# verdurin/pbdagcon

Hardware: AMD Instinct MI355X
Metric: consensus bases/sec (whole node) (higher is better)
Workload: dtype u8

## Files before the change

### include/dagcon.h

```cpp
#ifndef DAGCON_H
#define DAGCON_H

#include <stddef.h>
#include <stdint.h>

#ifdef __cplusplus
extern "C" {
#endif

#define DAGCON_ABI_VERSION 2

typedef enum dagcon_status {
    DAGCON_OK = 0,
    DAGCON_ERR_INVALID_ARG = -1,
    DAGCON_ERR_NO_DEVICE = -2,
    DAGCON_ERR_HIP = -3,
    DAGCON_ERR_NONCONFORMING = -4,
    DAGCON_ERR_UNSUPPORTED = -5,
    DAGCON_ERR_WORKSPACE = -6,
    DAGCON_ERR_INTERNAL = -7,
    DAGCON_ERR_STATE = -8
} dagcon_status;

#define DAGCON_MAX_COVERAGE 4094u
// ... 305 lines not shown
int dagcon_debug_counters(dagcon_ctx *ctx, unsigned long long *out8);

uint32_t dagcon_align_dropped(dagcon_ctx *ctx);

int dagcon_align_ends(dagcon_ctx *ctx, uint32_t n, uint32_t *q_begin, uint32_t *q_end, uint32_t *t_begin,
                      uint32_t *t_end);

#define DAGCON_PLACE_MAX_LEN 65536u
int dagcon_place(dagcon_ctx *ctx, const uint64_t *seq_off, const uint32_t *seq_len, const char *blob, uint64_t bytes,
                 uint32_t n_pairs, const uint32_t *pair_q, const uint32_t *pair_t, uint32_t k, uint32_t max_occ,
                 uint32_t *votes_fwd, uint32_t *votes_rev, char *strand, uint32_t *t0, uint32_t *t1);

int dagcon_debug_plan(uint32_t n_targets, uint64_t n_alignments, uint64_t sum_positions, uint32_t partial_span,
                      uint32_t max_segments, uint32_t min_segment_len, uint32_t out4[4]);

#ifdef __cplusplus
}
#endif
#endif
```

### pbdagcon_amd/capi.py

```python
from __future__ import annotations

import ctypes as C
import os

import numpy as np

_HERE = os.path.dirname(os.path.abspath(__file__))
LIB_PATH = os.path.join(_HERE, "libdagcon_hip.so")

DAGCON_OK = 0
ERR_NAMES = {
    -1: "DAGCON_ERR_INVALID_ARG", -2: "DAGCON_ERR_NO_DEVICE", -3: "DAGCON_ERR_HIP",
    -4: "DAGCON_ERR_NONCONFORMING", -5: "DAGCON_ERR_UNSUPPORTED", -6: "DAGCON_ERR_WORKSPACE",
    -7: "DAGCON_ERR_INTERNAL", -8: "DAGCON_ERR_STATE",
}
FLAG_RAW_ALIGNMENTS = 1
FLAG_STOP_AFTER_BUILD = 2
FLAG_STOP_AFTER_MERGE = 4
FLAG_DEBUG_RESWEEP = 16
FLAG_LOCAL_ALIGN = 32
FLAG_BASE_SUPPORT = 64
FLAG_BASE_POS = 256
MAX_COVERAGE = 4094
PLACE_MAX_LEN = 65536
# ... 5 lines not shown
    "dagcon_debug_counters", "dagcon_host_alloc", "dagcon_host_free", "dagcon_align",
    "dagcon_consensus_pre", "dagcon_debug_plan", "dagcon_align_dropped", "dagcon_align_panels",
    "dagcon_align_ends", "dagcon_place", "dagcon_fetch_support", "dagcon_upload_cigar", "dagcon_consensus_cigar",
    "dagcon_fetch_positions", "dagcon_upload_cigar_windows", "dagcon_consensus_cigar_windows",
    "dagcon_upload_cigar_packed", "dagcon_consensus_cigar_packed",
    "dagcon_upload_cigar_strand", "dagcon_consensus_cigar_strand",
    "dagcon_upload_cs", "dagcon_consensus_cs",
    "dagcon_set_record_filter", "dagcon_fetch_record_stats",
    "dagcon_set_edits", "dagcon_fetch_edits",
    "dagcon_set_edit_support", "dagcon_fetch_edit_support",
    "dagcon_set_pileup", "dagcon_fetch_pileup", "dagcon_fetch_pileup_sites",
    "dagcon_set_site_reads", "dagcon_fetch_site_reads",
    "dagcon_set_site_alleles", "dagcon_fetch_site_alleles", "dagcon_allele_text",
    "dagcon_set_hap_consensus", "dagcon_fetch_hap_tally", "dagcon_upload_haps", "dagcon_fetch_hap_map",
    "dagcon_upload_cigar_md", "dagcon_consensus_cigar_md", "dagcon_fetch_md_targets",
]
ABI_VERSION = 2


class DagconError(RuntimeError):
    def __init__(self, code, msg):
        super().__init__(f"{ERR_NAMES.get(code, code)}: {msg}")
        self.code = code


class Opts(C.Structure):
    _fields_ = [("min_cov", C.c_uint32), ("min_len", C.c_uint32), ("trim", C.c_uint32),
                ("min_weight", C.c_int32), ("device", C.c_int32), ("flags", C.c_uint32),
                ("max_segments", C.c_uint32), ("min_segment_len", C.c_uint32)]

# ... 191 lines not shown
    L.dagcon_fetch_pileup.argtypes = [vp, C.POINTER(Pileup)]
    L.dagcon_fetch_pileup_sites.argtypes = [vp, C.POINTER(PileupSites)]
    L.dagcon_set_site_reads.argtypes = [vp, C.POINTER(SiteReadsOpts)]
    L.dagcon_fetch_site_reads.argtypes = [vp, C.POINTER(SiteReads)]
    L.dagcon_set_site_alleles.argtypes = [vp, C.c_int]
    L.dagcon_fetch_site_alleles.argtypes = [vp, C.POINTER(SiteAlleles)]
    L.dagcon_allele_text.argtypes = [C.c_uint64, C.c_char_p, C.c_size_t]
    L.dagcon_set_hap_consensus.argtypes = [vp, C.POINTER(HapOpts)]
    L.dagcon_fetch_hap_tally.argtypes = [vp, C.POINTER(HapTally)]
    L.dagcon_upload_haps.argtypes = [vp]
    L.dagcon_fetch_hap_map.argtypes = [vp, C.POINTER(HapMap)]
    L.dagcon_upload_cigar_md.argtypes = [vp, C.POINTER(CigarBatch), C.POINTER(Windows), C.POINTER(MdTags), C.c_int]
    L.dagcon_consensus_cigar_md.argtypes = [vp, C.POINTER(CigarBatch), C.POINTER(Windows), C.POINTER(MdTags), C.c_int,
                                            C.POINTER(Results)]
    L.dagcon_fetch_md_targets.argtypes = [vp, C.POINTER(vp), C.POINTER(C.c_uint64)]
    L.dagcon_host_alloc.argtypes = [vp, C.c_size_t, C.POINTER(vp)]
    L.dagcon_host_free.argtypes = [vp, vp]
    L.dagcon_host_free.restype = None
    _LIB = L
    return L


def allele_text(key) -> str:
    buf = C.create_string_buffer(24)
    r = load().dagcon_allele_text(int(key), buf, 24)
    if r != 0:
        raise DagconError(r, "dagcon_allele_text: %#x is no key" % int(key))
    return buf.value.decode()


def default_opts() -> Opts:
    o = Opts()
    load().dagcon_default_opts(C.byref(o))
    return o


class HostBatch:

    def __init__(self, tlen, aln_begin, aln_start, aln_off, aln_len, qstr, tstr,
                 backbone=None, backbone_off=None, ids=None):
        self.tlen = np.ascontiguousarray(tlen, dtype=np.uint32)
        self.aln_begin = np.ascontiguousarray(aln_begin, dtype=np.uint64)
        self.aln_start = np.ascontiguousarray(aln_start, dtype=np.uint32)
# ... 623 lines not shown
        return {"src_target": np.ctypeslib.as_array(hm.src_target, shape=(T,)).copy() if T else np.zeros(0, np.uint32),
                "label": np.ctypeslib.as_array(hm.label, shape=(T,)).copy() if T else np.zeros(0, np.uint8),
                "aln_begin": begin,
                "aln_src": np.ctypeslib.as_array(hm.aln_src, shape=(n,)).copy() if n else np.zeros(0, np.uint64)}

    def edits(self) -> dict:
        e = Edits()
        self._chk(self.L.dagcon_fetch_edits(self.h, C.byref(e)))
        S, n = int(e.n_segments), int(e.n)

        def arr(ptr, k, dt):
            return np.ctypeslib.as_array(ptr, shape=(k,)).copy() if k else np.zeros(0, dt)
        return {"seg_t0": arr(e.seg_t0, S, np.uint32), "seg_t1": arr(e.seg_t1, S, np.uint32),
                "edit_begin": arr(e.edit_begin, S + 1, np.uint64), "t_pos": arr(e.t_pos, n, np.uint32),
                "t_len": arr(e.t_len, n, np.uint32), "c_off": arr(e.c_off, n, np.uint64), "c_len": arr(e.c_len, n, np.uint32)}

    def timings(self) -> dict:
        t = Timings()
        self._chk(self.L.dagcon_get_timings(self.h, C.byref(t)))
        return {k: getattr(t, k) for k, _ in Timings._fields_ if k != "reserved"}

    def normalize(self, alns, trim=0, raw=False):
        n = len(alns)
        starts = np.array([a[0] for a in alns], dtype=np.uint32)
        lens = np.array([len(a[1]) for a in alns], dtype=np.uint32)
        offs = np.zeros(n, dtype=np.uint64)
        if n:
            offs[1:] = np.cumsum(lens[:-1], dtype=np.uint64)
        q = np.frombuffer(b"".join(a[1] for a in alns) or b"\0", dtype=np.uint8)
        t = np.frombuffer(b"".join(a[2] for a in alns) or b"\0", dtype=np.uint8)
# ... 151 lines not shown
```

### pbdagcon_amd/csrc/api_ctx.h

```cpp
namespace {

struct Ctx;

struct DevBuf {
    void *p = nullptr;
    size_t cap = 0;
    DevBuf() = default;
    DevBuf(const DevBuf &) = delete;
    DevBuf &operator=(const DevBuf &) = delete;
    ~DevBuf() { release(); }
    void release() {
        if (p) (void)hipFree(p);
        p = nullptr; cap = 0;
    }
    template <class X> X *as() const { return static_cast<X *>(p); }
};

struct PinBuf {
    void *p = nullptr;
    size_t cap = 0;
    PinBuf() = default;
    PinBuf(const PinBuf &) = delete;
    PinBuf &operator=(const PinBuf &) = delete;
    ~PinBuf() { if (p) (void)hipHostFree(p); }
// ... 106 lines not shown
    uint32_t max_k = 0, max_tlen = 0;
    uint64_t sum_len = 0, sum_bb = 0, mat_cells = 0, blob_bytes = 0;
    bool have_bb = false;
    std::vector<uint32_t> h_tlen, h_aln_len, h_aln_start, h_aln_tgt;
    std::vector<uint64_t> h_aln_begin, h_aln_off, h_mat_base, h_bbv_base, h_bb_off, h_matc_base;
    std::vector<uint32_t> h_matc_stride;
    uint64_t matc_cells = 0;
    bool wide_cells = false;
    std::vector<uint8_t> h_tactive;
    std::vector<uint32_t> h_ch_base, h_ch_aln;
    std::vector<uint64_t> h_norm_off;
    std::vector<uint32_t> h_ck_base;
    uint64_t n_ckpt = 0;
    uint32_t emit_shift = 9;
    uint32_t n_chunks = 0;
    uint64_t tmp_main = 0, tmp_cap = 0;
    bool tmp_shared = false;

    InBufs in;
    RunBufs run;
    ArenaBufs arena;
    AlignBufs al;
    PanelBufs pn;
    PlaceBufs pl;
    CsBufs cs;
    CigarBufs cg;
    MdBufs md;
    bool md_valid = false, md_fetched = false;
    uint64_t md_bytes = 0;
    std::vector<char> h_md_t;
// ... 175 lines not shown
```

### pbdagcon_amd/csrc/api_run.hip.h

```cpp
namespace {

#define DQ_KMAX 52u
struct DgPlanIn { uint32_t T; uint64_t n_alns, sum_bb; uint32_t gcuts, max_segments, min_segment_len, seg_env, merge_q; };
struct DgPlan { uint32_t seg_max, seg_min, use_q, bp_max; };
static DgPlan dg_plan_pieces(const DgPlanIn &in) {
    DgPlan pl;
    const uint32_t T = in.T;
    pl.seg_min = in.min_segment_len;
    if (!pl.seg_min) pl.seg_min = (uint32_t)std::min<uint64_t>(768, std::max<uint64_t>(192, in.sum_bb / 8192));
    if (in.max_segments) pl.seg_max = in.max_segments > 64u ? 64u : in.max_segments;
    else if (in.seg_env) pl.seg_max = in.seg_env;
    else if (in.gcuts) pl.seg_max = 64;
    else { uint32_t sm = T ? 8192u / T : 8u; pl.seg_max = sm < 8u ? 8u : sm > 256u ? 256u : sm; }
    if (in.gcuts && !in.min_segment_len) pl.seg_min = 256;
    pl.use_q = 0;
    if (in.merge_q && !in.gcuts && pl.seg_max != 1) {
        const uint32_t slots = 1024u * DQ_WAVES;
        if (in.max_segments || in.seg_env) pl.use_q = 1;
        else if (T && in.n_alns <= (uint64_t)DQ_KMAX * T) {
            const uint64_t avail = std::min<uint64_t>(256, std::max<uint64_t>(1, in.sum_bb / T / 128));
            const uint64_t k = (uint64_t)T * avail / DQ_ROWS / slots;
            if (k >= 1 || (uint64_t)T * avail / DQ_ROWS * 10u >= 6u * slots) {
                const uint64_t sm = std::min<uint64_t>(avail, std::max<uint64_t>(k, 1) * slots * DQ_ROWS / T);
                if (sm >= 2) { pl.seg_max = (uint32_t)sm; pl.use_q = 1; }
            }
        }
    }
    if (pl.seg_max < 1) pl.seg_max = 1;
    if (pl.use_q && !in.min_segment_len) pl.seg_min = 128;
    pl.bp_max = pl.seg_max == 1 ? 1u : std::min(in.gcuts || T >= 256u ? 64u : (uint32_t)DG_BP_PIECES, 3u * pl.seg_max);
    if (pl.bp_max < 1) pl.bp_max = 1;
    return pl;
}

size_t seg_stride(const Ctx *c) { return ((size_t)c->seg_cap + 3) & ~(size_t)3; }

bool matc_wide(const Ctx *c) { return c->max_k > 64u || c->wide_cells; }
size_t matc_bytes(const Ctx *c) { return (size_t)c->matc_cells * (matc_wide(c) ? 4u : 1u); }

int ensure_stat(Ctx *c, uint32_t T) {
    StatBlock &b = c->sb;
    auto up16 = [](size_t x) { return (x + 15) & ~(size_t)15; };
    b.o_tfail = up16(sizeof(DgStatus));
    b.o_cns_len = b.o_tfail + up16(((size_t)T + 1) * 4);
    b.o_n_seg = b.o_cns_len + up16((size_t)T * 4);
    b.zero_bytes = b.o_n_seg + up16((size_t)T * 4);
    b.o_cns_off = b.zero_bytes;
// ... 99 lines not shown
    p.bb_off = c->in.bb_off.as<const uint64_t>();
    p.mat_base = c->in.mat_base.as<const uint64_t>();
    p.matc_base = c->in.matc_base.as<const uint64_t>(); p.matc_stride = c->in.matc_stride.as<const uint32_t>();
    p.bbv_base = c->in.bbv_base.as<const uint64_t>();
    p.T = c->T; p.A = c->A;
    p.trim = c->opts.trim; p.min_len = c->opts.min_len;
    p.min_weight = c->opts.min_weight < 0 ? (int32_t)c->opts.min_cov : c->opts.min_weight;
    p.flags = c->opts.flags;
    p.max_k = c->max_k; p.max_tlen = c->max_tlen;
    p.nmis = c->run.nmis.as<uint32_t>(); p.norm_off = c->in.norm_off.as<uint64_t>();
    p.n_lo = c->run.n_lo.as<uint32_t>(); p.n_hi = c->run.n_hi.as<uint32_t>();
    p.n_start = c->run.n_start.as<uint32_t>(); p.n_ins = c->run.n_ins.as<uint32_t>();
    p.n_del = c->run.n_del.as<uint32_t>();
    p.norm = c->arena.norm.as<uint16_t>(); p.norm_cap = c->norm_cap;
    p.ch_aln = c->in.ch_aln.as<const uint32_t>(); p.ch_base = c->in.ch_base.as<const uint32_t>();
    p.n_chunks = c->n_chunks;
    p.ch_k0 = c->run.ch_k0.as<uint32_t>(); p.ch_next = c->run.ch_next.as<uint32_t>();
    p.ch_w = c->run.ch_w.as<uint32_t>(); p.ch_tb = c->run.ch_tb.as<uint32_t>();
    p.ch_flag = c->run.ch_flag.as<uint32_t>(); p.ch_src = c->run.ch_src.as<uint64_t>();
    p.ch_out = c->run.ch_out.as<uint32_t>(); p.ch_adv = c->run.ch_adv.as<uint32_t>();
    p.n_lb = c->run.n_lb.as<uint32_t>(); p.norm_tmp = c->run.norm_tmp.as<uint16_t>();
    p.tmp_main = c->tmp_main; p.tmp_cap = c->tmp_cap; p.tmp_off = c->tmp_shared ? c->in.tmp_off.as<const uint64_t>() : nullptr;
    p.ckpt = c->run.ckpt.as<uint32_t>(); p.ck_base = c->in.ck_base.as<const uint32_t>(); p.emit_shift = c->emit_shift;
    p.node_base = c->run.node_base.as<uint64_t>(); p.n_nodes = c->run.n_nodes.as<uint32_t>();
    p.pool_base = c->run.pool_base.as<uint64_t>(); p.pool_size = c->run.pool_size.as<uint32_t>();
    p.pool_top = c->run.pool_top.as<uint32_t>(); p.t_nins = c->run.t_nins.as<uint32_t>();
    p.matA = c->arena.matA.as<uint32_t>(); p.matD = c->arena.matD.as<uint32_t>(); p.matC = c->arena.matC.p;
    p.cov = c->run.cov.as<int32_t>(); p.gcount = c->run.gcount.as<uint32_t>();
    p.gbase = c->run.gbase.as<uint32_t>(); p.bid = c->run.bid.as<uint32_t>();
    p.nodes = c->arena.nodes.as<DgNode>(); p.best = c->run.best.as<int32_t>();
    p.queue = c->run.queue.as<int32_t>(); p.score = c->run.score.as<float2>(); p.bp_tt = c->run.bp_tt.as<float>();
// ... 256 lines not shown
    c->device = opts->device;
    if (const char *e = getenv("DAGCON_EMIT_SHIFT")) {
        const int v = atoi(e);
        if (v >= 4 && v <= 20) c->emit_shift = (uint32_t)v;
    }
    if (const char *e = getenv("DAGCON_MERGE_SEGS")) {
        const int v = atoi(e);
        if (v >= 1 && v <= 64) c->seg_env = (uint32_t)v;
    }
    if (const char *e = getenv("DAGCON_FOLD")) c->fold = atoi(e) != 0;
    if (const char *e = getenv("DAGCON_POISON")) c->poison = atoi(e);
    if (const char *e = getenv("DAGCON_BP_LANE")) c->bp_lane = atoi(e);
    if (const char *e = getenv("DAGCON_BP_LANE_STACK")) c->bl_stk = atoi(e);
    if (const char *e = getenv("DAGCON_MERGE_Q")) c->merge_q = atoi(e) != 0;
    if (const char *e = getenv("DAGCON_EDITS_CAP")) c->ed_cap_env = atol(e);
    memset(&c->tm, 0, sizeof c->tm);
    memset(&c->h_st, 0, sizeof c->h_st);
    if (hipSetDevice(c->device) != hipSuccess || hipStreamCreateWithFlags(&c->stream, hipStreamNonBlocking) != hipSuccess) {
        delete c;
        return DAGCON_ERR_NO_DEVICE;
    }
    for (auto &e : c->ev)
        if (hipEventCreate(&e) != hipSuccess) { delete c; return DAGCON_ERR_HIP; }
    if (ensure_stat(c, 0) != DAGCON_OK) { delete c; return DAGCON_ERR_WORKSPACE; }
    *out = reinterpret_cast<dagcon_ctx *>(c);
    return DAGCON_OK;
}

void dagcon_destroy(dagcon_ctx *ctx) { delete reinterpret_cast<Ctx *>(ctx); }

static bool has_long_gap_run(const char *tstr, const std::vector<uint64_t> &off, const std::vector<uint32_t> &len) {
    for (size_t a = 0; a < len.size(); a++) {
        const char *s = tstr + off[a];
        uint32_t run = 0;
        for (uint32_t i = 0; i < len[a]; i++) {
            run = s[i] == '-' || s[i] == '.' ? run + 1 : 0;
            if (run > 255u) return true;
        }
    }
// ... 75 lines not shown
        c->sum_bb += ((uint64_t)b->tlen[t] + 2 + 3) & ~3ull;
        if (c->have_bb) {
            c->h_bb_off[t] = b->backbone_off[t];
            bb_bytes = std::max<uint64_t>(bb_bytes, b->backbone_off[t] + b->tlen[t]);
        }
    }
    if (was_wide && !dev_t && b->tstr) c->wide_cells = has_long_gap_run(b->tstr, c->h_aln_off, c->h_aln_len);
    c->full_span = n_whole == (uint64_t)c->h_aln_len.size();
    c->gcuts = c->full_span ? 0u : 1u;
    if (const char *e = getenv("DAGCON_GCUTS")) c->gcuts = atoi(e) ? 1u : 0u;
    {
        DgPlanIn pi;
        pi.T = T; pi.n_alns = c->h_aln_len.size(); pi.sum_bb = c->sum_bb; pi.gcuts = c->gcuts;
        pi.max_segments = c->opts.max_segments; pi.min_segment_len = c->opts.min_segment_len;
        pi.seg_env = c->seg_env; pi.merge_q = c->merge_q ? 1u : 0u;
        const DgPlan pl = dg_plan_pieces(pi);
        c->seg_max = pl.seg_max; c->seg_min = pl.seg_min; c->use_q = (int)pl.use_q; c->bp_max = pl.bp_max;
    }
    if (const char *e = getenv("DAGCON_BP_SEGS")) { const int v = atoi(e); if (v >= 1 && v <= 64) c->bp_max = (uint32_t)v; }
    {
        const uint64_t pieces = std::max<uint64_t>(1, (uint64_t)T * std::max(c->bp_max, c->seg_max));
        const uint32_t fit = (uint32_t)std::min<uint64_t>(4096, (512ull << 20) / pieces);
        const uint32_t base = std::max(256u, fit);
        if (c->stk_words < base || (uint64_t)c->stk_words * pieces > (1024ull << 20)) c->stk_words = base;
    }
    if (c->gcuts) c->worklist_cap = std::max<uint32_t>(c->worklist_cap, (uint32_t)std::min<uint64_t>((uint64_t)T * c->seg_max + 64, 0x0FFFFFFFull));
    c->h_aln_begin[T] = c->h_aln_len.size();
    if (c->h_aln_len.size() > 0xFFFFFFF0ull) return fail(c, DAGCON_ERR_UNSUPPORTED, "too many alignments");
    c->A = (uint32_t)c->h_aln_len.size();
    c->blob_bytes = b->blob_bytes;
    c->h_ch_base.assign((size_t)c->A + 1, 0);
    c->h_ch_aln.clear();
    for (uint32_t a = 0; a < c->A; a++) {
        const uint32_t nw = std::max<uint32_t>(1u, (c->h_aln_len[a] + DG_NCH - 1) / DG_NCH);
        c->h_ch_base[a] = (uint32_t)c->h_ch_aln.size();
        if (c->h_ch_aln.size() + nw > 0xFFFFFFF0ull) return fail(c, DAGCON_ERR_UNSUPPORTED, "too many alignment columns");
        c->h_ch_aln.insert(c->h_ch_aln.end(), nw, a);
    }
    c->h_norm_off.assign((size_t)c->A, 0);
    {
        uint64_t top = 0;
        for (uint32_t a = 0; a < c->A; a++) { c->h_norm_off[a] = top; top += (2ull * c->h_aln_len[a] + 7ull) & ~7ull; }
        c->norm_cap = std::max<uint64_t>(c->norm_cap, top + 64);
    }
    c->h_ck_base.assign((size_t)c->A, 0);
    c->n_ckpt = 0;
    for (uint32_t a = 0; a < c->A; a++) {
        c->h_ck_base[a] = (uint32_t)c->n_ckpt;
        c->n_ckpt += (((uint64_t)c->h_tlen[c->h_aln_tgt[a]] + 2) >> c->emit_shift) + 1;
// ... 763 lines not shown
    if (!ctx || !out8) return DAGCON_ERR_INVALID_ARG;
    for (int i = 0; i < 16; i++) out8[i] = 0;
    return DAGCON_OK;
}

uint32_t dagcon_align_dropped(dagcon_ctx *ctx) {
    return ctx ? reinterpret_cast<Ctx *>(ctx)->align_dropped : 0u;
}

int dagcon_debug_plan(uint32_t n_targets, uint64_t n_alignments, uint64_t sum_positions, uint32_t partial_span,
                      uint32_t max_segments, uint32_t min_segment_len, uint32_t out4[4]) {
    if (!out4) return DAGCON_ERR_INVALID_ARG;
    DgPlanIn pi;
    pi.T = n_targets; pi.n_alns = n_alignments; pi.sum_bb = sum_positions; pi.gcuts = partial_span ? 1u : 0u;
    pi.max_segments = max_segments; pi.min_segment_len = min_segment_len; pi.seg_env = 0; pi.merge_q = 1;
    const DgPlan pl = dg_plan_pieces(pi);
    out4[0] = pl.seg_max; out4[1] = pl.seg_min; out4[2] = pl.use_q; out4[3] = pl.bp_max;
    return DAGCON_OK;
}

int dagcon_get_timings(dagcon_ctx *ctx, dagcon_timings *out) {
    if (!ctx || !out) return DAGCON_ERR_INVALID_ARG;
    Ctx *c = reinterpret_cast<Ctx *>(ctx);
    if (!c->ran) return fail(c, DAGCON_ERR_STATE, "no run to report");
    if (!c->fetched) {
        HIPCHK(c, hipSetDevice(c->device));
        HIPCHK(c, hipStreamSynchronize(c->stream));
        if (int r = read_timings(c)) return r;
    }
    *out = c->tm;
    return DAGCON_OK;
}
// ... 83 lines not shown
```

### pbdagcon_amd/csrc/dagcon_dev.h

```cpp
#pragma once
#include <hip/hip_runtime.h>
#include <stdint.h>

#define DG_GAP '-'

#define DG_F_RAW      1u
#define DG_F_A1_ONLY  8u
#define DG_F_RESWEEP  16u

#define DG_E_BADCHAR     0x001u
#define DG_E_NONCONF     0x002u
#define DG_E_NORM_OVF    0x004u
#define DG_E_NODE_OVF    0x008u
#define DG_E_POOL_OVF    0x010u
#define DG_E_POOL_TGT    0x020u
#define DG_E_STACK       0x040u
#define DG_E_INTERNAL    0x080u
#define DG_E_OUT_OVF     0x100u
#define DG_E_TOO_BIG     0x200u
#define DG_E_LOG_OVF     0x800u
#define DG_E_LIST_OVF    0x400u
#define DG_E_RUN_WIDE    0x1000u
#define DG_E_ED_OVF      0x2000u
#define DG_E_SITE_OVF    0x4000u
// ... 53 lines not shown
    const uint64_t *mat_base;
    const uint64_t *bbv_base;
    uint32_t T, A;
    uint32_t trim, min_len;
    int32_t min_weight;
    uint32_t flags;
    uint32_t max_k, max_tlen;
    uint32_t *nmis;
    uint64_t *norm_off;
    uint32_t *n_lo, *n_hi, *n_start, *n_ins, *n_del;
    uint16_t *norm;
    uint64_t norm_cap;
    const uint32_t *ch_aln;
    const uint32_t *ch_base;
    uint32_t n_chunks;
    uint32_t *ch_k0;
    uint32_t *ch_next;
    uint32_t *ch_w, *ch_tb;
    uint32_t *ch_flag;
    uint64_t *ch_src;
    uint32_t *ch_out, *ch_adv;
    uint32_t *n_lb;
    uint16_t *norm_tmp;
    uint32_t *ckpt;
    const uint32_t *ck_base;
    uint32_t emit_shift;
    uint64_t tmp_main, tmp_cap;
    const uint64_t *tmp_off;
    uint64_t *node_base;
    uint32_t *n_nodes;
// ... 144 lines not shown
```

### pbdagcon_amd/csrc/k_bestpath.hip.h

```cpp
#pragma once
#include <hip/hip_runtime.h>
#include <float.h>
#include <type_traits>
#include "dagcon_dev.h"

#define DG_TT_TEN 1.0e30f
__global__ __launch_bounds__(256) void k_bp_terms(DgParams p) {
    const uint32_t t = blockIdx.x;
    if (dg_failed(p) || dg_tskip(p, t)) return;
    const uint64_t nb = p.node_base[t];
    const uint32_t N = p.n_nodes[t];
    const int32_t *cov = p.cov + p.bbv_base[t];
    const DgNode *nd = p.nodes + nb;
    for (uint32_t v = blockIdx.y * 256 + threadIdx.x; v < N; v += gridDim.y * 256) {
        const uint4 h = *reinterpret_cast<const uint4 *>(&nd[v]);
        const uint4 h2 = *(reinterpret_cast<const uint4 *>(&nd[v]) + 1);
        float tt;
        if (((h.y >> 8) & DG_NF_BACKBONE) && (int)h.z == 1) tt = DG_TT_TEN;
        else tt = (float)cov[(int)h2.w] * 0.5f;
        p.bp_tt[nb + v] = tt;
        p.score[nb + v] = make_float2(0.0f, 0.0f);
        p.best[nb + v] = -1;
    }
}
// ... 419 lines not shown
    const float a = p.score[nb + P.c_bot].x;
    if (lane == 0) { p.bp_stat[2 * (uint64_t)blockIdx.x] = amax; p.bp_stat[2 * (uint64_t)blockIdx.x + 1] = a; }
}

#define DG_BL_STK 16
#define DG_BRW 8
#define DG_BRR 32
#define DG_BRP 8
__device__ __forceinline__ uint32_t dbr_ballot(bool q) { return (uint32_t)((__ballot(q) >> (threadIdx.x & (64u - DG_BRW))) & 0xffull); }
__device__ __forceinline__ float dbr_max(float m) {
    m = fmaxf(m, __int_as_float(__builtin_amdgcn_update_dpp(0, __float_as_int(m), 0xB1, 0xf, 0xf, true)));
    m = fmaxf(m, __int_as_float(__builtin_amdgcn_update_dpp(0, __float_as_int(m), 0x4E, 0xf, 0xf, true)));
    m = fmaxf(m, __int_as_float(__builtin_amdgcn_update_dpp(0, __float_as_int(m), 0x141, 0xf, 0xf, true)));
    return m;
}
__global__ __launch_bounds__(64) void k_bp_sweep_l(DgParams p) {
    constexpr int ROWS = 64 / DG_BRW;
    __shared__ int s_stk[ROWS * DG_BL_STK];
    __shared__ int s_rtag[ROWS * DG_BRR];
    __shared__ float s_rsc[ROWS * DG_BRR], s_rtt[ROWS * DG_BRR];
    __shared__ int s_pid[ROWS * DG_BRP], s_pbd[ROWS * DG_BRP];
    __shared__ float s_pmx[ROWS * DG_BRP];
    if (dg_failed(p)) return;
    const int l = threadIdx.x & (DG_BRW - 1);
    const uint32_t row = threadIdx.x / DG_BRW;
    const uint32_t piece = blockIdx.x * (uint32_t)ROWS + row;
    const uint32_t t = piece / p.bp_max, seg = piece % p.bp_max;
    if (t >= p.T || dg_tskip(p, t)) return;
    const uint32_t *crow = p.cuts_bp + (uint64_t)t * (p.bp_max + 2u);
    const uint32_t nseg = crow[0];
    if (seg >= nseg) return;
    const uint64_t nb = p.node_base[t];
    const DgNode *nd = p.nodes + nb;
    float2 *score = p.score + nb;
    int32_t *best = p.best + nb;
    const uint32_t *pool = p.pool + p.pool_base[t];
    const float *tt = p.bp_tt + nb;
    const int N = (int)p.n_nodes[t];
    const int c_bot = (int)crow[1 + seg];
    const int c_top = seg + 1 < nseg ? (int)crow[2 + seg] : -1;
    const int v_top = c_top >= 0 ? c_top - 1 : N - 1;
    int *stk = s_stk + row * DG_BL_STK;
    int *rtag = s_rtag + row * DG_BRR;
    float *rsc = s_rsc + row * DG_BRR, *rtt = s_rtt + row * DG_BRR;
    int *pid = s_pid + row * DG_BRP, *pbd = s_pbd + row * DG_BRP;
    float *pmx = s_pmx + row * DG_BRP;
    for (int i = l; i < DG_BRR; i += DG_BRW) rtag[i] = -1;
    const int stk_cap = (int)p.bl_stk;
    float amax = 0.0f;
    int bad = 0;
    uint32_t guard = 0;
    const uint32_t guard_max = 64u * (uint32_t)(v_top - c_bot + 1) + 1000000u;
    const char *g_base = reinterpret_cast<const char *>(nd) + ((l == 1 || l >= 5) ? 4 : l == 2 ? 16 : 0);
    uint32_t g_shift = 5;
    if (l == 3) { g_base = reinterpret_cast<const char *>(score) + 4; g_shift = 3; }
    if (l == 4) { g_base = reinterpret_cast<const char *>(tt); g_shift = 2; }
    const int g_back = l >= 5 ? l - 4 : 0;
#define DBR_GATHER(X, OUT)                                                                               \
    do {                                                                                                 \
        const int xl_ = (X) - g_back;                                                                    \
        OUT = *reinterpret_cast<const uint32_t *>(g_base + ((uint64_t)(uint32_t)(xl_ < 0 ? 0 : xl_) << g_shift)); \
// ... 609 lines not shown
```

### pbdagcon_amd/csrc/k_build.hip.h

```cpp
#pragma once
#include <hip/hip_runtime.h>
#include "dagcon_dev.h"
#include "k_norm_run.hip.h"
#include "k_norm_fin.hip.h"

#define DG_WAVE 64
#ifndef DG_LPW
#define DG_LPW 8u
#endif

__device__ __forceinline__ bool dg_failed(const DgParams &p) {
    return __hip_atomic_load(&p.st->err_flags, __ATOMIC_RELAXED, __HIP_MEMORY_SCOPE_AGENT) != 0;
}
__device__ __forceinline__ void dg_fail(const DgParams &p, uint32_t bit) {
    atomicOr(&p.st->err_flags, bit);
}
__device__ __forceinline__ void dg_fail_target(const DgParams &p, uint32_t t, uint32_t bit) {
    atomicOr(&p.tfail[t], bit);
}
__device__ __forceinline__ bool dg_tskip(const DgParams &p, uint32_t t) {
    return !p.tactive[t] || __hip_atomic_load(&p.tfail[t], __ATOMIC_RELAXED, __HIP_MEMORY_SCOPE_AGENT) != 0;
}
__device__ __forceinline__ bool dg_askip(const DgParams &p, uint32_t a) {
    return !(p.flags & DG_F_A1_ONLY) && __hip_atomic_load(&p.tfail[p.aln_tgt[a]], __ATOMIC_RELAXED, __HIP_MEMORY_SCOPE_AGENT) != 0;
// ... 87 lines not shown
    if (RETRY && p.ch_flag[g] != 2u) return;
    const uint32_t a = p.ch_aln[g];
    if (dg_askip(p, a)) { if (!RETRY) p.ch_flag[g] = 0; return; }
    const uint32_t c = g - p.ch_base[a], nwin = p.ch_base[a + 1] - p.ch_base[a];
    const uint64_t off = p.aln_off[a];
    const uint32_t len = p.aln_len[a];
    const uint8_t *q = p.q + off, *t = p.t + off;
    uint32_t flag = 0;
    DgChunkRun r;
    r.w = 0; r.tb = 0; r.dirty = false; r.overflow = false; r.badchar = false;
    uint32_t k0 = DG_CH_NONE, cn = c + 1;
    uint64_t src = 0;
    if (p.flags & DG_F_RAW) {
        if (c == 0) { k0 = 0; cn = nwin; flag = 1; }
    } else {
        k0 = dg_chunk_start(q, t, len, c);
        if (k0 != DG_CH_NONE) {
            uint16_t *win = s_win + threadIdx.x * (NW + 2u);
            const uint64_t soff = p.tmp_off ? p.tmp_off[a] : off;
            src = (2ull * (soff + k0) + 8ull * g + 7ull) & ~7ull;
            for (;;) {
                uint32_t k1 = len;
                for (; cn < nwin; cn++) {
                    const uint32_t s = dg_chunk_start(q, t, len, cn);
                    if (s != DG_CH_NONE) { k1 = s; break; }
                }
                if constexpr (NW == DG_NW) r = dg_norm_run_gc(q, t, len, k0, k1, win, p.norm_tmp + src);
                else r = dg_norm_run<NW>(q, t, len, k0, k1, win, p.norm_tmp + src);
                if (r.badchar) dg_fail_aln(p, a, DG_E_BADCHAR);
                if (r.overflow) { flag = RETRY ? 1u : 2u; break; }
                if (!r.dirty) break;
                cn++;
                uint32_t k2 = len;
                for (uint32_t x = cn; x < nwin; x++) {
                    const uint32_t s = dg_chunk_start(q, t, len, x);
                    if (s != DG_CH_NONE) { k2 = s; break; }
                }
                const unsigned long long need = (2ull * (k2 - k0) + 15ull) & ~7ull;
                const unsigned long long o = atomicAdd(&p.st->ovf_top, need);
                if (p.tmp_main + o + need > p.tmp_cap) { flag = 1; break; }
                src = p.tmp_main + o;
            }
        }
    }
    p.ch_k0[g] = k0; p.ch_next[g] = cn; p.ch_w[g] = r.w; p.ch_tb[g] = r.tb;
    p.ch_flag[g] = flag; p.ch_src[g] = src;
}

__global__ __launch_bounds__(64) void k_norm_scan(DgParams p) {
    const uint32_t a = blockIdx.x * 64 + threadIdx.x;
// ... 1123 lines not shown
```

### pbdagcon_amd/csrc/k_norm_run.hip.h

```cpp
#pragma once
#include <stddef.h>
#include <stdint.h>

#if defined(__HIPCC__)
#include <hip/hip_runtime.h>
#define DG_HD __host__ __device__
#define DG_HD_INLINE __host__ __device__ __forceinline__
typedef uint4 dg_u4;
#define DG_MAKE_U4(a, b, c, d) make_uint4((a), (b), (c), (d))
#else
#define DG_HD
#define DG_HD_INLINE inline __attribute__((always_inline))
struct __attribute__((may_alias, aligned(16))) dg_u4 { uint32_t x, y, z, w; };
static inline dg_u4 DG_MAKE_U4(uint32_t a, uint32_t b, uint32_t c, uint32_t d) { dg_u4 v; v.x = a; v.y = b; v.z = c; v.w = d; return v; }
#endif
#ifndef DG_GAP
#define DG_GAP '-'
#endif

#define DG_COL(qb, tb) ((uint16_t)((uint16_t)(qb) | ((uint16_t)(tb) << 8)))
#define DG_Q(c) ((uint8_t)((c) & 0xff))
#define DG_T(c) ((uint8_t)((c) >> 8))

#ifndef DG_NCH
#define DG_NCH 512u
#endif
#define DG_CH_NONE 0xFFFFFFFFu

DG_HD_INLINE bool dg_match_col(uint8_t qb, uint8_t tb) { return qb == tb && qb != DG_GAP && qb != '.'; }

DG_HD inline uint32_t dg_chunk_start(const uint8_t *q, const uint8_t *t, uint32_t len, uint32_t c) {
    if (c == 0) return 0;
    const uint64_t w0 = (uint64_t)c * DG_NCH;
    if (w0 >= len) return DG_CH_NONE;
    const uint32_t hi = (uint64_t)len < w0 + DG_NCH ? len : (uint32_t)(w0 + DG_NCH);
    for (uint32_t k = (uint32_t)w0; k < hi; k++) {
        const uint8_t b = q[k];
        if (dg_match_col(b, t[k]) && b != q[k - 1] && dg_match_col(q[k - 1], t[k - 1]) && dg_match_col(q[k - 2], t[k - 2]))
            return k;
    }
    return DG_CH_NONE;
}

struct DgChunkRun { uint32_t w, tb; bool dirty, overflow, badchar; };

template <uint32_t NW>
DG_HD inline DgChunkRun dg_norm_run(const uint8_t *q, const uint8_t *t, const uint32_t len, const uint32_t k0,
                                    const uint32_t k1, uint16_t *win, uint16_t *out) {
#define DG_W(x) win[(x) & (NW - 1u)]
    DgChunkRun r;
    r.w = 0; r.tb = 0; r.dirty = false; r.overflow = false; r.badchar = false;
    if (k0 >= k1) return r;
    uint32_t badw = 0;
    uint32_t ip = k0, e = 0, i = 0, w = 0, tb = 0, jt = 0, jq = 0;
    uint32_t e_end = 0xFFFFFFFFu;
    uint32_t o0 = 0, o1 = 0, o2 = 0, o3 = 0;
// ... 253 lines not shown
```

Measured before the change: 382.7 million.

## Size normalization chunks and planner slots from queried device occupancy

Queries the CU count and per-kernel resident waves at context creation and feeds them into the segment and best-path planners in place of hard-coded slot counts. It adds a best-path piece cap tied to resident sweep slots. The normalization chunk length is now picked per batch by a cost model that trades chunk length against wave rounds. k_bp_sweep_l gets a waves-per-EU attribute and a per-row shared-memory struct, and the chunk length becomes a runtime parameter for the device kernels. The aim is less tail idling and better fill across the whole GPU, at the risk of less inlined constant-length loops and different plan choices.

Result: no change. 383.9 million, median of 4 (+0.3%).

```diff
diff --git a/include/dagcon.h b/include/dagcon.h
--- a/include/dagcon.h
+++ b/include/dagcon.h
@@ -343,6 +343,10 @@
 int dagcon_debug_plan(uint32_t n_targets, uint64_t n_alignments, uint64_t sum_positions, uint32_t partial_span,
                       uint32_t max_segments, uint32_t min_segment_len, uint32_t out4[4]);
 
+int dagcon_debug_chunk_len(const uint32_t *aln_len, uint32_t n, uint32_t slots, uint32_t out3[3]);
+
+int dagcon_debug_residency(dagcon_ctx *ctx, uint32_t out8[8]);
+
 #ifdef __cplusplus
 }
 #endif
diff --git a/pbdagcon_amd/capi.py b/pbdagcon_amd/capi.py
--- a/pbdagcon_amd/capi.py
+++ b/pbdagcon_amd/capi.py
@@ -43,6 +43,7 @@
     "dagcon_set_site_alleles", "dagcon_fetch_site_alleles", "dagcon_allele_text",
     "dagcon_set_hap_consensus", "dagcon_fetch_hap_tally", "dagcon_upload_haps", "dagcon_fetch_hap_map",
     "dagcon_upload_cigar_md", "dagcon_consensus_cigar_md", "dagcon_fetch_md_targets",
+    "dagcon_debug_chunk_len", "dagcon_debug_residency",
 ]
 ABI_VERSION = 2
 
@@ -264,6 +265,8 @@
     L.dagcon_consensus_cigar_md.argtypes = [vp, C.POINTER(CigarBatch), C.POINTER(Windows), C.POINTER(MdTags), C.c_int,
                                             C.POINTER(Results)]
     L.dagcon_fetch_md_targets.argtypes = [vp, C.POINTER(vp), C.POINTER(C.c_uint64)]
+    L.dagcon_debug_chunk_len.argtypes = [vp, C.c_uint32, C.c_uint32, C.POINTER(C.c_uint32)]
+    L.dagcon_debug_residency.argtypes = [vp, C.POINTER(C.c_uint32)]
     L.dagcon_host_alloc.argtypes = [vp, C.c_size_t, C.POINTER(vp)]
     L.dagcon_host_free.argtypes = [vp, vp]
     L.dagcon_host_free.restype = None
@@ -277,6 +280,15 @@
     if r != 0:
         raise DagconError(r, "dagcon_allele_text: %#x is no key" % int(key))
     return buf.value.decode()
+
+
+def chunk_len(aln_len, slots):
+    a = np.ascontiguousarray(aln_len, dtype=np.uint32)
+    o = (C.c_uint32 * 3)()
+    r = load().dagcon_debug_chunk_len(a.ctypes.data if a.size else None, int(a.size), int(slots), o)
+    if r != 0:
+        raise DagconError(r, "dagcon_debug_chunk_len")
+    return int(o[0]), int(o[1]), int(o[2])
 
 
 def default_opts() -> Opts:
@@ -930,6 +942,12 @@
         return {"seg_t0": arr(e.seg_t0, S, np.uint32), "seg_t1": arr(e.seg_t1, S, np.uint32),
                 "edit_begin": arr(e.edit_begin, S + 1, np.uint64), "t_pos": arr(e.t_pos, n, np.uint32),
                 "t_len": arr(e.t_len, n, np.uint32), "c_off": arr(e.c_off, n, np.uint64), "c_len": arr(e.c_len, n, np.uint32)}
+
+    def residency(self) -> dict:
+        o = (C.c_uint32 * 8)()
+        self._chk(self.L.dagcon_debug_residency(self.h, o))
+        return {"k_merge_q": o[0], "k_bp_sweep_l": o[1], "k_bp_walk_r": o[2], "k_norm_chunk": o[3], "k_emit": o[4],
+                "cus": o[5], "bp_max": o[6], "norm_chunk": o[7]}
 
     def timings(self) -> dict:
         t = Timings()
diff --git a/pbdagcon_amd/csrc/api_ctx.h b/pbdagcon_amd/csrc/api_ctx.h
--- a/pbdagcon_amd/csrc/api_ctx.h
+++ b/pbdagcon_amd/csrc/api_ctx.h
@@ -144,6 +144,8 @@
     uint64_t n_ckpt = 0;
     uint32_t emit_shift = 9;
     uint32_t n_chunks = 0;
+    uint32_t nch = DG_NCH, nch_env = 0;
+    uint32_t resident[5] = {4u * DQ_WAVES, 32u, 32u, 19u, 20u}, n_cu = 256, bp_slots_env = 0;
     uint64_t tmp_main = 0, tmp_cap = 0;
     bool tmp_shared = false;
 
diff --git a/pbdagcon_amd/csrc/api_run.hip.h b/pbdagcon_amd/csrc/api_run.hip.h
--- a/pbdagcon_amd/csrc/api_run.hip.h
+++ b/pbdagcon_amd/csrc/api_run.hip.h
@@ -1,7 +1,13 @@
 namespace {
 
 #define DQ_KMAX 52u
-struct DgPlanIn { uint32_t T; uint64_t n_alns, sum_bb; uint32_t gcuts, max_segments, min_segment_len, seg_env, merge_q; };
+struct DgPlanIn { uint32_t T; uint64_t n_alns, sum_bb; uint32_t gcuts, max_segments, min_segment_len, seg_env, merge_q;
+                  uint32_t slots_wave, slots_q, slots_bp, bp_hold; };
+#define DG_NOM_CUS 256u
+static void dg_plan_nominal(DgPlanIn &in) {
+    in.slots_wave = DG_NOM_CUS * 32u; in.slots_q = DG_NOM_CUS * 4u * DQ_WAVES; in.slots_bp = DG_NOM_CUS * 32u; in.bp_hold = 0;
+}
+enum { DG_RES_MERGE_Q = 0, DG_RES_BP_SWEEP_L, DG_RES_BP_WALK_R, DG_RES_NORM_CHUNK, DG_RES_EMIT, DG_RES_N };
 struct DgPlan { uint32_t seg_max, seg_min, use_q, bp_max; };
 static DgPlan dg_plan_pieces(const DgPlanIn &in) {
     DgPlan pl;
@@ -11,11 +17,11 @@
     if (in.max_segments) pl.seg_max = in.max_segments > 64u ? 64u : in.max_segments;
     else if (in.seg_env) pl.seg_max = in.seg_env;
     else if (in.gcuts) pl.seg_max = 64;
-    else { uint32_t sm = T ? 8192u / T : 8u; pl.seg_max = sm < 8u ? 8u : sm > 256u ? 256u : sm; }
+    else { uint32_t sm = T ? in.slots_wave / T : 8u; pl.seg_max = sm < 8u ? 8u : sm > 256u ? 256u : sm; }
     if (in.gcuts && !in.min_segment_len) pl.seg_min = 256;
     pl.use_q = 0;
     if (in.merge_q && !in.gcuts && pl.seg_max != 1) {
-        const uint32_t slots = 1024u * DQ_WAVES;
+        const uint32_t slots = std::max(1u, in.slots_q);
         if (in.max_segments || in.seg_env) pl.use_q = 1;
         else if (T && in.n_alns <= (uint64_t)DQ_KMAX * T) {
             const uint64_t avail = std::min<uint64_t>(256, std::max<uint64_t>(1, in.sum_bb / T / 128));
@@ -29,8 +35,40 @@
     if (pl.seg_max < 1) pl.seg_max = 1;
     if (pl.use_q && !in.min_segment_len) pl.seg_min = 128;
     pl.bp_max = pl.seg_max == 1 ? 1u : std::min(in.gcuts || T >= 256u ? 64u : (uint32_t)DG_BP_PIECES, 3u * pl.seg_max);
+    if (in.bp_hold && !in.gcuts && T) {
+        const uint64_t hold = (uint64_t)in.slots_bp * 8u / T;
+        if (hold < pl.bp_max) pl.bp_max = (uint32_t)hold;
+    }
     if (pl.bp_max < 1) pl.bp_max = 1;
     return pl;
+}
+
+#define DG_NCH_MIN 256u
+#define DG_NCH_MAX (DG_FIN_NP * 512u * 7u / 8u / 64u * 64u)
+#define DG_NCH_C0 174u
+struct DgChunkPlan { uint32_t len, waves, rounds; };
+static uint64_t dg_chunk_waves(const uint32_t *aln_len, const size_t n, const uint32_t L) {
+    uint64_t chunks = 0;
+    for (size_t a = 0; a < n; a++) chunks += std::max<uint64_t>(1, ((uint64_t)aln_len[a] + L - 1) / L);
+    return (chunks + 63) / 64;
+}
+static DgChunkPlan dg_plan_chunk_len(const uint32_t *aln_len, const size_t n, uint32_t slots) {
+    if (slots < 1) slots = 1;
+    auto plan = [&](const uint32_t L) {
+        const uint64_t w = dg_chunk_waves(aln_len, n, L);
+        DgChunkPlan pl;
+        pl.len = L; pl.waves = (uint32_t)std::min<uint64_t>(w, 0xFFFFFFFFull); pl.rounds = (uint32_t)std::min<uint64_t>((w + slots - 1) / slots, 0xFFFFFFFFull);
+        return pl;
+    };
+    DgChunkPlan best = plan(DG_NCH);
+    if (best.rounds <= 1) return best;
+    uint64_t cost = (uint64_t)best.rounds * (DG_NCH + DG_NCH_C0);
+    for (uint32_t L = DG_NCH_MIN; L <= DG_NCH_MAX; L += 64u) {
+        const DgChunkPlan pl = plan(L);
+        const uint64_t cl = (uint64_t)pl.rounds * (L + DG_NCH_C0);
+        if (cl < cost || (cl == cost && L < best.len)) { best = pl; cost = cl; }
+    }
+    return best;
 }
 
 size_t seg_stride(const Ctx *c) { return ((size_t)c->seg_cap + 3) & ~(size_t)3; }
@@ -160,7 +198,7 @@
     p.n_del = c->run.n_del.as<uint32_t>();
     p.norm = c->arena.norm.as<uint16_t>(); p.norm_cap = c->norm_cap;
     p.ch_aln = c->in.ch_aln.as<const uint32_t>(); p.ch_base = c->in.ch_base.as<const uint32_t>();
-    p.n_chunks = c->n_chunks;
+    p.n_chunks = c->n_chunks; p.nch = c->nch;
     p.ch_k0 = c->run.ch_k0.as<uint32_t>(); p.ch_next = c->run.ch_next.as<uint32_t>();
     p.ch_w = c->run.ch_w.as<uint32_t>(); p.ch_tb = c->run.ch_tb.as<uint32_t>();
     p.ch_flag = c->run.ch_flag.as<uint32_t>(); p.ch_src = c->run.ch_src.as<uint64_t>();
@@ -447,6 +485,14 @@
     if (const char *e = getenv("DAGCON_BP_LANE_STACK")) c->bl_stk = atoi(e);
     if (const char *e = getenv("DAGCON_MERGE_Q")) c->merge_q = atoi(e) != 0;
     if (const char *e = getenv("DAGCON_EDITS_CAP")) c->ed_cap_env = atol(e);
+    if (const char *e = getenv("DAGCON_NORM_CHUNK")) {
+        const long v = atol(e);
+        if (v >= 16 && v <= 0x40000000l && v % 16 == 0) c->nch_env = (uint32_t)v;
+    }
+    if (const char *e = getenv("DAGCON_BP_SLOTS")) {
+        const long v = atol(e);
+        if (v >= 1 && v <= 0x40000000l) c->bp_slots_env = (uint32_t)v;
+    }
     memset(&c->tm, 0, sizeof c->tm);
     memset(&c->h_st, 0, sizeof c->h_st);
     if (hipSetDevice(c->device) != hipSuccess || hipStreamCreateWithFlags(&c->stream, hipStreamNonBlocking) != hipSuccess) {
@@ -456,6 +502,21 @@
     for (auto &e : c->ev)
         if (hipEventCreate(&e) != hipSuccess) { delete c; return DAGCON_ERR_HIP; }
     if (ensure_stat(c, 0) != DAGCON_OK) { delete c; return DAGCON_ERR_WORKSPACE; }
+    {
+        hipDeviceProp_t prop;
+        if (hipGetDeviceProperties(&prop, c->device) == hipSuccess && prop.multiProcessorCount > 0) c->n_cu = (uint32_t)prop.multiProcessorCount;
+        auto ask = [&](const int which, const void *k, const int block) {
+            int nb = 0;
+            if (hipOccupancyMaxActiveBlocksPerMultiprocessor(&nb, k, block, 0) == hipSuccess && nb > 0)
+                c->resident[which] = (uint32_t)nb * (uint32_t)((block + 63) / 64);
+            else (void)hipGetLastError();
+        };
+        ask(DG_RES_MERGE_Q, reinterpret_cast<const void *>(&k_merge_q), 64);
+        ask(DG_RES_BP_SWEEP_L, reinterpret_cast<const void *>(&k_bp_sweep_l), 64);
+        ask(DG_RES_BP_WALK_R, reinterpret_cast<const void *>(&k_bp_walk_r<false, false>), 64);
+        ask(DG_RES_NORM_CHUNK, reinterpret_cast<const void *>(&k_norm_chunk<DG_NW, 64, false>), 64);
+        ask(DG_RES_EMIT, reinterpret_cast<const void *>(&k_emit<uint8_t>), 64);
+    }
     *out = reinterpret_cast<dagcon_ctx *>(c);
     return DAGCON_OK;
 }
@@ -561,6 +622,8 @@
         pi.T = T; pi.n_alns = c->h_aln_len.size(); pi.sum_bb = c->sum_bb; pi.gcuts = c->gcuts;
         pi.max_segments = c->opts.max_segments; pi.min_segment_len = c->opts.min_segment_len;
         pi.seg_env = c->seg_env; pi.merge_q = c->merge_q ? 1u : 0u;
+        pi.slots_wave = c->n_cu * 32u; pi.slots_q = c->n_cu * c->resident[DG_RES_MERGE_Q];
+        pi.slots_bp = c->bp_slots_env ? c->bp_slots_env : c->n_cu * c->resident[DG_RES_BP_SWEEP_L]; pi.bp_hold = 1;
         const DgPlan pl = dg_plan_pieces(pi);
         c->seg_max = pl.seg_max; c->seg_min = pl.seg_min; c->use_q = (int)pl.use_q; c->bp_max = pl.bp_max;
     }
@@ -576,10 +639,12 @@
     if (c->h_aln_len.size() > 0xFFFFFFF0ull) return fail(c, DAGCON_ERR_UNSUPPORTED, "too many alignments");
     c->A = (uint32_t)c->h_aln_len.size();
     c->blob_bytes = b->blob_bytes;
+    c->nch = c->nch_env ? c->nch_env
+                        : dg_plan_chunk_len(c->h_aln_len.data(), c->A, c->n_cu * c->resident[DG_RES_NORM_CHUNK]).len;
     c->h_ch_base.assign((size_t)c->A + 1, 0);
     c->h_ch_aln.clear();
     for (uint32_t a = 0; a < c->A; a++) {
-        const uint32_t nw = std::max<uint32_t>(1u, (c->h_aln_len[a] + DG_NCH - 1) / DG_NCH);
+        const uint32_t nw = (uint32_t)std::max<uint64_t>(1u, ((uint64_t)c->h_aln_len[a] + c->nch - 1) / c->nch);
         c->h_ch_base[a] = (uint32_t)c->h_ch_aln.size();
         if (c->h_ch_aln.size() + nw > 0xFFFFFFF0ull) return fail(c, DAGCON_ERR_UNSUPPORTED, "too many alignment columns");
         c->h_ch_aln.insert(c->h_ch_aln.end(), nw, a);
@@ -1373,8 +1438,24 @@
     DgPlanIn pi;
     pi.T = n_targets; pi.n_alns = n_alignments; pi.sum_bb = sum_positions; pi.gcuts = partial_span ? 1u : 0u;
     pi.max_segments = max_segments; pi.min_segment_len = min_segment_len; pi.seg_env = 0; pi.merge_q = 1;
+    dg_plan_nominal(pi);
     const DgPlan pl = dg_plan_pieces(pi);
     out4[0] = pl.seg_max; out4[1] = pl.seg_min; out4[2] = pl.use_q; out4[3] = pl.bp_max;
+    return DAGCON_OK;
+}
+
+int dagcon_debug_chunk_len(const uint32_t *aln_len, uint32_t n, uint32_t slots, uint32_t out3[3]) {
+    if (!out3 || (n && !aln_len)) return DAGCON_ERR_INVALID_ARG;
+    const DgChunkPlan pl = dg_plan_chunk_len(aln_len, n, slots);
+    out3[0] = pl.len; out3[1] = pl.waves; out3[2] = pl.rounds;
+    return DAGCON_OK;
+}
+
+int dagcon_debug_residency(dagcon_ctx *ctx, uint32_t out8[8]) {
+    if (!ctx || !out8) return DAGCON_ERR_INVALID_ARG;
+    const Ctx *c = reinterpret_cast<const Ctx *>(ctx);
+    for (int i = 0; i < DG_RES_N; i++) out8[i] = c->resident[i];
+    out8[5] = c->n_cu; out8[6] = c->uploaded ? c->bp_max : 0u; out8[7] = c->uploaded ? c->nch : 0u;
     return DAGCON_OK;
 }
 
diff --git a/pbdagcon_amd/csrc/dagcon_dev.h b/pbdagcon_amd/csrc/dagcon_dev.h
--- a/pbdagcon_amd/csrc/dagcon_dev.h
+++ b/pbdagcon_amd/csrc/dagcon_dev.h
@@ -91,6 +91,7 @@
     const uint32_t *ch_aln;
     const uint32_t *ch_base;
     uint32_t n_chunks;
+    uint32_t nch;
     uint32_t *ch_k0;
     uint32_t *ch_next;
     uint32_t *ch_w, *ch_tb;
diff --git a/pbdagcon_amd/csrc/k_bestpath.hip.h b/pbdagcon_amd/csrc/k_bestpath.hip.h
--- a/pbdagcon_amd/csrc/k_bestpath.hip.h
+++ b/pbdagcon_amd/csrc/k_bestpath.hip.h
@@ -457,13 +457,16 @@
     m = fmaxf(m, __int_as_float(__builtin_amdgcn_update_dpp(0, __float_as_int(m), 0x141, 0xf, 0xf, true)));
     return m;
 }
-__global__ __launch_bounds__(64) void k_bp_sweep_l(DgParams p) {
+__global__ __launch_bounds__(64) __attribute__((amdgpu_waves_per_eu(8, 8))) void k_bp_sweep_l(DgParams p) {
     constexpr int ROWS = 64 / DG_BRW;
-    __shared__ int s_stk[ROWS * DG_BL_STK];
-    __shared__ int s_rtag[ROWS * DG_BRR];
-    __shared__ float s_rsc[ROWS * DG_BRR], s_rtt[ROWS * DG_BRR];
-    __shared__ int s_pid[ROWS * DG_BRP], s_pbd[ROWS * DG_BRP];
-    __shared__ float s_pmx[ROWS * DG_BRP];
+    struct Row {
+        int stk[DG_BL_STK];
+        int rtag[DG_BRR];
+        float rsc[DG_BRR], rtt[DG_BRR];
+        int pid[DG_BRP], pbd[DG_BRP];
+        float pmx[DG_BRP];
+    };
+    __shared__ Row s_row[ROWS];
     if (dg_failed(p)) return;
     const int l = threadIdx.x & (DG_BRW - 1);
     const uint32_t row = threadIdx.x / DG_BRW;
@@ -483,11 +486,12 @@
     const int c_bot = (int)crow[1 + seg];
     const int c_top = seg + 1 < nseg ? (int)crow[2 + seg] : -1;
     const int v_top = c_top >= 0 ? c_top - 1 : N - 1;
-    int *stk = s_stk + row * DG_BL_STK;
-    int *rtag = s_rtag + row * DG_BRR;
-    float *rsc = s_rsc + row * DG_BRR, *rtt = s_rtt + row * DG_BRR;
-    int *pid = s_pid + row * DG_BRP, *pbd = s_pbd + row * DG_BRP;
-    float *pmx = s_pmx + row * DG_BRP;
+    Row &R = s_row[row];
+    int *stk = R.stk;
+    int *rtag = R.rtag;
+    float *rsc = R.rsc, *rtt = R.rtt;
+    int *pid = R.pid, *pbd = R.pbd;
+    float *pmx = R.pmx;
     for (int i = l; i < DG_BRR; i += DG_BRW) rtag[i] = -1;
     const int stk_cap = (int)p.bl_stk;
     float amax = 0.0f;
diff --git a/pbdagcon_amd/csrc/k_build.hip.h b/pbdagcon_amd/csrc/k_build.hip.h
--- a/pbdagcon_amd/csrc/k_build.hip.h
+++ b/pbdagcon_amd/csrc/k_build.hip.h
@@ -125,7 +125,7 @@
     if (p.flags & DG_F_RAW) {
         if (c == 0) { k0 = 0; cn = nwin; flag = 1; }
     } else {
-        k0 = dg_chunk_start(q, t, len, c);
+        k0 = dg_chunk_start_n(q, t, len, c, p.nch);
         if (k0 != DG_CH_NONE) {
             uint16_t *win = s_win + threadIdx.x * (NW + 2u);
             const uint64_t soff = p.tmp_off ? p.tmp_off[a] : off;
@@ -133,7 +133,7 @@
             for (;;) {
                 uint32_t k1 = len;
                 for (; cn < nwin; cn++) {
-                    const uint32_t s = dg_chunk_start(q, t, len, cn);
+                    const uint32_t s = dg_chunk_start_n(q, t, len, cn, p.nch);
                     if (s != DG_CH_NONE) { k1 = s; break; }
                 }
                 if constexpr (NW == DG_NW) r = dg_norm_run_gc(q, t, len, k0, k1, win, p.norm_tmp + src);
@@ -144,7 +144,7 @@
                 cn++;
                 uint32_t k2 = len;
                 for (uint32_t x = cn; x < nwin; x++) {
-                    const uint32_t s = dg_chunk_start(q, t, len, x);
+                    const uint32_t s = dg_chunk_start_n(q, t, len, x, p.nch);
                     if (s != DG_CH_NONE) { k2 = s; break; }
                 }
                 const unsigned long long need = (2ull * (k2 - k0) + 15ull) & ~7ull;
diff --git a/pbdagcon_amd/csrc/k_norm_run.hip.h b/pbdagcon_amd/csrc/k_norm_run.hip.h
--- a/pbdagcon_amd/csrc/k_norm_run.hip.h
+++ b/pbdagcon_amd/csrc/k_norm_run.hip.h
@@ -29,17 +29,20 @@
 
 DG_HD_INLINE bool dg_match_col(uint8_t qb, uint8_t tb) { return qb == tb && qb != DG_GAP && qb != '.'; }
 
-DG_HD inline uint32_t dg_chunk_start(const uint8_t *q, const uint8_t *t, uint32_t len, uint32_t c) {
+DG_HD inline uint32_t dg_chunk_start_n(const uint8_t *q, const uint8_t *t, uint32_t len, uint32_t c, uint32_t nch) {
     if (c == 0) return 0;
-    const uint64_t w0 = (uint64_t)c * DG_NCH;
+    const uint64_t w0 = (uint64_t)c * nch;
     if (w0 >= len) return DG_CH_NONE;
-    const uint32_t hi = (uint64_t)len < w0 + DG_NCH ? len : (uint32_t)(w0 + DG_NCH);
+    const uint32_t hi = (uint64_t)len < w0 + nch ? len : (uint32_t)(w0 + nch);
     for (uint32_t k = (uint32_t)w0; k < hi; k++) {
         const uint8_t b = q[k];
         if (dg_match_col(b, t[k]) && b != q[k - 1] && dg_match_col(q[k - 1], t[k - 1]) && dg_match_col(q[k - 2], t[k - 2]))
             return k;
     }
     return DG_CH_NONE;
+}
+DG_HD inline uint32_t dg_chunk_start(const uint8_t *q, const uint8_t *t, uint32_t len, uint32_t c) {
+    return dg_chunk_start_n(q, t, len, c, DG_NCH);
 }
 
 struct DgChunkRun { uint32_t w, tb; bool dirty, overflow, badchar; };
```
